# ox-vgg/wise

Measured on AMD Instinct MI355X. Metric: frames/sec embedded (ViT-B/32 bs=256) + queries/sec over 10M×512 index, 1/2/4/8 MI355X, higher is better.
Workload: dtype bf16; 1 GPU; OpenCLIP ViT-B/32 image tower (encode_image + L2 normalise), bs=256 frames per GPU, fp32 normalised frames resident in HBM -> [256,512] fp32 unit vectors; seeded random weights (no checkpoints offline); batches_in_flight=2, distinct_input_batches=4, layernorm_fold=True, global_batch=256, frames_per_gpu=256, parallelism=dp1, device=AMD Radeon Graphics

## Files before the change

### wise_amd/csrc/vit.hip

```cpp
#include "transformer.h"
#include "gemm_w4.h"

namespace wise {
#ifdef WISE_DEBUG_KNOBS
static int g_ablate = 0;
#else
constexpr int g_ablate = 0;
#endif

template <int NV>
__global__ __launch_bounds__(256) void layernorm_kernel(const float* x , const float* __restrict__ w,
                                                        const float* __restrict__ b, int rows, int W, float eps,
                                                        bf16_t* __restrict__ y, float* xo = nullptr) {
    const int lane = threadIdx.x & 63;
    const int row = blockIdx.x * 4 + (threadIdx.x >> 6);
    if (row >= rows) return;
    const int w4 = W >> 2;
    const float4* xr = reinterpret_cast<const float4*>(x + (size_t)row * W);
    float4 v[NV];
    float s = 0.f;
#pragma unroll
    for (int i = 0; i < NV; ++i) {
        const int c = i * 64 + lane;
        v[i] = (c < w4) ? xr[c] : make_float4(0.f, 0.f, 0.f, 0.f);
// ... 161 lines not shown
}

int layernorm_f32_dual(const float* x, const float* w, const float* b, int rows, int W, float eps, float* xo, bf16_t* y,
                       hipStream_t st) {
    WISE_CHECK_ARG(x && w && b && y && xo, "layernorm_dual: null pointer");
    WISE_CHECK_ARG(rows >= 0 && W > 128 && W % 4 == 0 && W <= 4096, "layernorm_dual: W=%d must be a multiple of 4 in (128, 4096]", W);
    if (rows == 0) return WISE_OK;
    const int nv = (W / 4 + 63) / 64;
    const dim3 grid((rows + 3) / 4), block(256);
#define LN_CASE(n) \
    case n: hipLaunchKernelGGL(layernorm_kernel<n>, grid, block, 0, st, x, w, b, rows, W, eps, y, xo); break;
    switch (nv) {
        LN_CASE(1) LN_CASE(2) LN_CASE(3) LN_CASE(4) LN_CASE(5) LN_CASE(6) LN_CASE(7) LN_CASE(8)
        LN_CASE(9) LN_CASE(10) LN_CASE(11) LN_CASE(12) LN_CASE(13) LN_CASE(14) LN_CASE(15) LN_CASE(16)
    }
#undef LN_CASE
    WISE_LAUNCH_CHECK("layernorm_kernel (dual)");
    return WISE_OK;
}

constexpr int V_RS = 144;
using short4v = __attribute__((ext_vector_type(4))) short;

template <int QT, bool MASK, int ND = 4>
__device__ __forceinline__ void softmax_block(f32x4 (&sacc)[4][QT], bf16x8 (&pf)[2][QT], f32x4 (&oacc)[ND][QT],
                                              float (&mrun)[QT], float (&lrun)[QT], int kbase, const int (&klim)[QT]) {
    const float sc = (ND == 4 ? 0.125f : 0.11180339887498948f) * 1.4426950408889634f;
#pragma unroll
    for (int qt = 0; qt < QT; ++qt) {
        float mx = -INFINITY;
#pragma unroll
        for (int kt = 0; kt < 4; ++kt)
#pragma unroll
            for (int r = 0; r < 4; ++r) {
                if (MASK && kbase + kt * 16 + r >= klim[qt]) sacc[kt][qt][r] = -INFINITY;
                mx = fmaxf(mx, sacc[kt][qt][r]);
            }
        mx = fmaxf(mx, __shfl_xor(mx, 16, 64));
        mx = fmaxf(mx, __shfl_xor(mx, 32, 64));
        const float mnew = fmaxf(mrun[qt], mx * sc);
        const float alpha = __builtin_amdgcn_exp2f(mrun[qt] - mnew);
        mrun[qt] = mnew;
        float ps = 0.f;
        float p[4][4];
#pragma unroll
        for (int kt = 0; kt < 4; ++kt)
#pragma unroll
            for (int r = 0; r < 4; ++r) {
                p[kt][r] = __builtin_amdgcn_exp2f(fmaf(sacc[kt][qt][r], sc, -mnew));
                ps += p[kt][r];
            }
        lrun[qt] = lrun[qt] * alpha + ps;
#pragma unroll
        for (int dt = 0; dt < ND; ++dt) {
            oacc[dt][qt][0] *= alpha; oacc[dt][qt][1] *= alpha;
            oacc[dt][qt][2] *= alpha; oacc[dt][qt][3] *= alpha;
        }
#pragma unroll
        for (int ks = 0; ks < 2; ++ks) {
            bf16x8 f;
#pragma unroll
            for (int r = 0; r < 4; ++r) {
                f[r] = (__bf16)p[2 * ks][r];
                f[4 + r] = (__bf16)p[2 * ks + 1][r];
            }
            pf[ks][qt] = f;
        }
    }
}

struct ClsRows {
    const bf16_t* hi = nullptr;
    long long lo_off = 0;
    bf16_t* hc = nullptr;
    long long lc_off = 0;
    const float* rs = nullptr;
    float* rs_c = nullptr;
    int* cnt = nullptr;
    int ncnt = 0;
};
__device__ __forceinline__ void cls_row_copy(const ClsRows& cr, int b, int T, int W, int lane) {
    const uint2* src = reinterpret_cast<const uint2*>(cr.hi + (size_t)b * T * W);
    uint2* dst = reinterpret_cast<uint2*>(cr.hc + (size_t)b * W);
    const long long so = cr.lo_off >> 2, dof = cr.lc_off >> 2;
    for (int c = lane; c < (W >> 2); c += 64) {
        dst[c] = src[c];
        dst[c + dof] = src[c + so];
    }
    if (cr.rs && lane == 0) cr.rs_c[b] = cr.rs[(size_t)b * T];
    if (b == 0)
        for (int c = lane; c < cr.ncnt; c += 64) cr.cnt[c] = 0;
}

template <int QT, bool CAUSAL, int DH = 64, bool PF = false, bool CLS = false>
__global__ __launch_bounds__(256, (QT == 2 && DH == 64 && !PF) ? 4 : 2) void attention_kernel(const bf16_t* __restrict__ qkv, int B, int T, int H,
                                                        bf16_t* __restrict__ o, const int* __restrict__ lens = nullptr,
                                                        const ClsRows cr = ClsRows()) {
    static_assert(!CLS || (QT == 1 && DH == 64 && !CAUSAL && !PF), "attention_kernel: the class-query form is QT = 1, DH = 64, no mask");
    constexpr int NS = (DH + 31) / 32, ND = DH / 16, VRS = DH * 2 + 16;
    __shared__ __attribute__((aligned(16))) unsigned char v_all[4][64 * VRS];
    const int lane = threadIdx.x & 63;
    const int wave = threadIdx.x >> 6;
    const int nqc = CLS ? 1 : (T + 16 * QT - 1) / (16 * QT);
    const long long item = (long long)blockIdx.x * 4 + wave;
    if (item >= (long long)B * H * nqc) return;
    const int qc = (int)(item % nqc);
    const int h = (int)((item / nqc) % H);
    const int b = (int)(item / ((long long)nqc * H));
    const int W = H * DH, W3 = 3 * W;
    const bf16_t* base = qkv + (size_t)b * T * W3;
    unsigned char* vimg = v_all[wave];
    const int l15 = lane & 15, g = lane >> 4;
    const int Tk = lens ? max(1, min(T, lens[b])) : T;

    const bf16x8 zero8 = {0, 0, 0, 0, 0, 0, 0, 0};
    bf16x8 qf[QT][NS];
#pragma unroll
    for (int qt = 0; qt < QT; ++qt) {
        int t = CLS ? 0 : qc * (16 * QT) + qt * 16 + l15;
        if (t >= T) t = T - 1;
#pragma unroll
        for (int s = 0; s < NS; ++s)
            qf[qt][s] = (s * 32 + g * 8 < DH) ? *reinterpret_cast<const bf16x8*>(base + (size_t)t * W3 + h * DH + s * 32 + g * 8)
                                              : zero8;
    }

    f32x4 oacc[ND][QT];
#pragma unroll
    for (int i = 0; i < ND; ++i)
#pragma unroll
        for (int j = 0; j < QT; ++j) oacc[i][j] = f32x4{0.f, 0.f, 0.f, 0.f};
    float mrun[QT], lrun[QT];
#pragma unroll
    for (int qt = 0; qt < QT; ++qt) { mrun[qt] = -INFINITY; lrun[qt] = 0.f; }

    const int q_last = min(T, (qc + 1) * (16 * QT)) - 1;
    const int nkb = CAUSAL ? (q_last >> 6) + 1 : (Tk + 63) >> 6;
    constexpr int CPR = DH / 8;
    auto load_k = [&](int kb, bf16x8 (&kf)[4][NS]) {
#pragma unroll
        for (int kt = 0; kt < 4; ++kt) {
            int t = kb * 64 + kt * 16 + l15;
            if (t >= Tk) t = Tk - 1;
#pragma unroll
            for (int s2 = 0; s2 < NS; ++s2)
                kf[kt][s2] = (s2 * 32 + g * 8 < DH) ? *reinterpret_cast<const bf16x8*>(base + (size_t)t * W3 + W + h * DH + s2 * 32 + g * 8)
                                                    : zero8;
        }
    };
    auto load_v = [&](int kb, uint4 (&vr)[CPR]) {
#pragma unroll
        for (int p = 0; p < CPR; ++p) {
            const int c = p * 64 + lane, key = c / CPR, part = c - key * CPR;
            int t = kb * 64 + key;
            const bool valid = t < Tk;
            if (!valid) t = Tk - 1;
            uint4 v = *reinterpret_cast<const uint4*>(base + (size_t)t * W3 + 2 * W + h * DH + part * 8);
            if (!valid) v = make_uint4(0u, 0u, 0u, 0u);
            vr[p] = v;
        }
// ... 57 lines not shown
            }
#pragma unroll
            for (int qt = 0; qt < QT; ++qt) {
                f32x4 c = f32x4{0.f, 0.f, 0.f, 0.f};
#pragma unroll
                for (int s2 = 0; s2 < NS; ++s2) c = __builtin_amdgcn_mfma_f32_16x16x32_bf16(kf[kt * KI][s2], qf[qt][s2], c, 0, 0, 0);
                sacc[kt][qt] = c;
            }
        }
        bf16x8 pf[2][QT];
        {
            int klim[QT];
#pragma unroll
            for (int qt = 0; qt < QT; ++qt) klim[qt] = CAUSAL ? min(T, qc * (16 * QT) + qt * 16 + l15 + 1) : Tk;
            if (CAUSAL || kb * 64 + 64 > Tk) {
#pragma unroll
                for (int qt = 0; qt < QT; ++qt)
#pragma unroll
                    for (int kt = 0; kt < 4; ++kt)
#pragma unroll
                        for (int r = 0; r < 4; ++r)
                            if (kb * 64 + kt * 16 + g * 4 + r >= klim[qt]) sacc[kt][qt][r] = -INFINITY;
            }
            softmax_block<QT, false, ND>(sacc, pf, oacc, mrun, lrun, kb * 64 + g * 4, klim);
        }
#pragma unroll
        for (int ks = 0; ks < 2; ++ks) {
#pragma unroll
            for (int dt = 0; dt < ND; ++dt) {
                const unsigned char* blk = vimg + (ks * 32 + g * 4 + (l15 >> 2)) * VRS + (dt * 16 + (l15 & 3) * 4) * 2;
                const short4v lo = __builtin_amdgcn_ds_read_tr16_b64_v4i16(
                    (__attribute__((address_space(3))) short4v*)(blk));
                const short4v hi = __builtin_amdgcn_ds_read_tr16_b64_v4i16(
                    (__attribute__((address_space(3))) short4v*)(blk + 16 * VRS));
                union { short8 s; bf16x8 f; } cv;
                cv.s = short8{lo[0], lo[1], lo[2], lo[3], hi[0], hi[1], hi[2], hi[3]};
#pragma unroll
                for (int qt = 0; qt < QT; ++qt)
                    oacc[dt][qt] = __builtin_amdgcn_mfma_f32_16x16x32_bf16(cv.f, pf[ks][qt], oacc[dt][qt], 0, 0, 0);
            }
        }
    }
#pragma unroll
    for (int qt = 0; qt < QT; ++qt) {
        float l = lrun[qt];
        l += __shfl_xor(l, 16, 64);
        l += __shfl_xor(l, 32, 64);
        const float inv = 1.f / l;
// ... 44 lines not shown
int attention_bf16(const bf16_t* qkv, int B, int T, int H, bf16_t* o, hipStream_t st, bool causal, int dh, const int* lens) {
    WISE_CHECK_ARG(qkv && o && B > 0 && T > 0 && H > 0, "attention: bad argument");
    WISE_CHECK_ARG(dh == 64 || (dh == 80 && !causal), "attention: head dim %d (64, or 80 without a mask)", dh);
    WISE_CHECK_ARG(!lens || (dh == 64 && !causal), "attention: per-sequence key counts go with head dim 64 and no causal mask");
    if (g_ablate & 4) return WISE_OK;
    if (dh == 80) {
        const long long items = (long long)B * H * ((T + 31) / 32);
        hipLaunchKernelGGL((attention_kernel<2, false, 80>), dim3((unsigned)((items + 3) / 4)), dim3(256), 0, st, qkv, B, T, H, o, (const int*)nullptr);
        WISE_LAUNCH_CHECK("attention_kernel");
        return WISE_OK;
    }
    if (!causal && g_attn_qt == 3) {
        const long long it3 = (long long)B * H * ((T + 47) / 48);
        hipLaunchKernelGGL((attention_kernel<3, false, 64, true>), dim3((unsigned)((it3 + 3) / 4)), dim3(256), 0, st, qkv, B, T, H, o, lens);
        WISE_LAUNCH_CHECK("attention_kernel");
        return WISE_OK;
    }
    if (!causal && g_attn_qt == 5) {
        const long long it2 = (long long)B * H * ((T + 31) / 32);
        hipLaunchKernelGGL((attention_kernel<2, false, 64, true>), dim3((unsigned)((it2 + 3) / 4)), dim3(256), 0, st, qkv, B, T, H, o, lens);
        WISE_LAUNCH_CHECK("attention_kernel");
        return WISE_OK;
    }
    const int qt = g_attn_qt ? (g_attn_qt == 4 ? 4 : 2) : (T <= 32 ? 2 : 4);
    const int nqc = (T + 16 * qt - 1) / (16 * qt);
    const long long items = (long long)B * H * nqc;
    const dim3 grid((unsigned)((items + 3) / 4)), block(256);
    if (causal) {
        if (qt == 4)
            hipLaunchKernelGGL((attention_kernel<4, true>), grid, block, 0, st, qkv, B, T, H, o, (const int*)nullptr);
        else
            hipLaunchKernelGGL((attention_kernel<2, true>), grid, block, 0, st, qkv, B, T, H, o, (const int*)nullptr);
    } else if (qt == 4)
        hipLaunchKernelGGL((attention_kernel<4, false>), grid, block, 0, st, qkv, B, T, H, o, lens);
    else
        hipLaunchKernelGGL((attention_kernel<2, false>), grid, block, 0, st, qkv, B, T, H, o, lens);
    WISE_LAUNCH_CHECK("attention_kernel");
    return WISE_OK;
}

#ifdef WISE_DEBUG_KNOBS
__device__ unsigned long long g_ao_stamps[12][8];
static int g_ao_dbg = 0;
#define AO_STAMP(k) do { if ((dbg & 8) && blockIdx.x == 0 && lane == 0) g_ao_stamps[wave][k] = __builtin_amdgcn_s_memtime(); } while (0)
#define AO_DBG_PARAM , int dbg
#define AO_DBG_ARG , g_ao_dbg
#else
#define AO_STAMP(k) do {} while (0)
#define AO_DBG_PARAM
#define AO_DBG_ARG
constexpr int dbg = 0;
#endif
template <int H>
__global__ __launch_bounds__(64 * H, 1) void attn_oproj_fold_kernel(const bf16_t* __restrict__ qkv, int T,
                                                                    const bf16_t* __restrict__ Wt, const float* __restrict__ bias,
                                                                    bf16_t* __restrict__ hi, long long lo_off,
// ... 379 lines not shown
#pragma unroll
                for (int e = 0; e < 4; ++e) {
                    acc[c8 * 8 + 2 * e] = fmaf(sc[i], __uint_as_float(w4[e] << 16), acc[c8 * 8 + 2 * e]);
                    acc[c8 * 8 + 2 * e + 1] = fmaf(sc[i], __uint_as_float(w4[e] & 0xFFFF0000u), acc[c8 * 8 + 2 * e + 1]);
                }
            }
        }
    }
    const float inv = 1.f / ps;
    float mine = 0.f;
#pragma unroll
    for (int j = 0; j < 64; ++j) {
        const float tot = wave_sum(acc[j]);
        if (lane == j) mine = tot * inv;
    }
    o[(size_t)b * W + h * 64 + lane] = f32_to_bf16(mine);
}

template <int NV>
__global__ __launch_bounds__(256) void embed_lnpre_kernel(const float* __restrict__ patch_out,
                                                          const float* __restrict__ cls, const float* __restrict__ pos,
                                                          const float* __restrict__ w, const float* __restrict__ bb,
                                                          int rows, int T, int W, float eps, float* __restrict__ x,
                                                          bf16_t* __restrict__ hcopy, float* __restrict__ rstd_out, long long lo_off) {
    const int lane = threadIdx.x & 63;
    const int row = blockIdx.x * 4 + (threadIdx.x >> 6);
    if (row >= rows) return;
    const int b = row / T, t = row % T;
    const int w4 = W >> 2;
    const float4* src = (t == 0) ? reinterpret_cast<const float4*>(cls)
                                 : reinterpret_cast<const float4*>(patch_out + ((size_t)b * (T - 1) + (t - 1)) * W);
    const float4* pr = reinterpret_cast<const float4*>(pos + (size_t)t * W);
    float4 v[NV];
    float s = 0.f;
#pragma unroll
    for (int i = 0; i < NV; ++i) {
        const int c = i * 64 + lane;
        if (c < w4) {
            float4 a = src[c], p = pr[c];
            v[i] = make_float4(a.x + p.x, a.y + p.y, a.z + p.z, a.w + p.w);
        } else
            v[i] = make_float4(0.f, 0.f, 0.f, 0.f);
        s += (v[i].x + v[i].y) + (v[i].z + v[i].w);
    }
    const float mean = wave_sum(s) / (float)W;
    float q = 0.f;
#pragma unroll
// ... 19 lines not shown
    }
    if (hcopy) {
        float s2 = 0.f;
#pragma unroll
        for (int i = 0; i < NV; ++i)
            if (i * 64 + lane < w4) s2 += (v[i].x + v[i].y) + (v[i].z + v[i].w);
        const float mean2 = wave_sum(s2) / (float)W;
        float q2 = 0.f;
#pragma unroll
        for (int i = 0; i < NV; ++i) {
            const int c = i * 64 + lane;
            if (c < w4) {
                float a0 = v[i].x - mean2, a1 = v[i].y - mean2, a2 = v[i].z - mean2, a3 = v[i].w - mean2;
                q2 += (a0 * a0 + a1 * a1) + (a2 * a2 + a3 * a3);
                const unsigned h0 = pack_bf16x2(v[i].x, v[i].y), h1 = pack_bf16x2(v[i].z, v[i].w);
                reinterpret_cast<uint2*>(hcopy + (size_t)row * W)[c] = make_uint2(h0, h1);
                reinterpret_cast<uint2*>(hcopy + lo_off + (size_t)row * W)[c] =
                    make_uint2(pack_bf16x2(v[i].x - __uint_as_float(h0 << 16), v[i].y - __uint_as_float(h0 & 0xffff0000u)),
                               pack_bf16x2(v[i].z - __uint_as_float(h1 << 16), v[i].w - __uint_as_float(h1 & 0xffff0000u)));
            }
        }
        const float r2 = rsqrtf(wave_sum(q2) / (float)W + eps);
        if (lane == 0) rstd_out[row] = r2;
    }
}

template <int NV>
__global__ __launch_bounds__(256) void cls_ln_kernel(const float* __restrict__ x, const float* __restrict__ w,
                                                     const float* __restrict__ b, int B, int T, int W, float eps,
                                                     bf16_t* __restrict__ y, const int* __restrict__ pos) {
    const int lane = threadIdx.x & 63;
    const int img = blockIdx.x * 4 + (threadIdx.x >> 6);
    if (img >= B) return;
    const int w4 = W >> 2;
    const float4* xr = reinterpret_cast<const float4*>(x + ((size_t)img * T + (pos ? pos[img] : 0)) * W);
    float4 v[NV];
    float s = 0.f;
#pragma unroll
    for (int i = 0; i < NV; ++i) {
        const int c = i * 64 + lane;
        v[i] = (c < w4) ? xr[c] : make_float4(0.f, 0.f, 0.f, 0.f);
        s += (v[i].x + v[i].y) + (v[i].z + v[i].w);
    }
    const float mean = wave_sum(s) / (float)W;
    float q = 0.f;
#pragma unroll
    for (int i = 0; i < NV; ++i) {
        if (i * 64 + lane < w4) {
            float a0 = v[i].x - mean, a1 = v[i].y - mean, a2 = v[i].z - mean, a3 = v[i].w - mean;
            q += (a0 * a0 + a1 * a1) + (a2 * a2 + a3 * a3);
        }
    }
    const float rstd = rsqrtf(wave_sum(q) / (float)W + eps);
    uint2* yr = reinterpret_cast<uint2*>(y + (size_t)img * W);
#pragma unroll
    for (int i = 0; i < NV; ++i) {
        const int c = i * 64 + lane;
        if (c < w4) {
            const float4 ww = reinterpret_cast<const float4*>(w)[c];
            const float4 bb = reinterpret_cast<const float4*>(b)[c];
            uint2 pk;
            pk.x = pack_bf16x2((v[i].x - mean) * rstd * ww.x + bb.x, (v[i].y - mean) * rstd * ww.y + bb.y);
            pk.y = pack_bf16x2((v[i].z - mean) * rstd * ww.z + bb.z, (v[i].w - mean) * rstd * ww.w + bb.w);
            yr[c] = pk;
// ... 36 lines not shown
    int rc;
    if (L > 0 && (rc = layernorm_f32_bf16(x, bw.pf + bw.ln1_w, bw.pf + bw.ln1_b, M, W, eps, h, st))) return rc;
    for (int l = 0; l < L; ++l) {
        const bf16_t* lwb = bw.wb + bw.per_layer_b * l;
        const float* lpf = bw.pf + bw.per_layer_f * l;
        if ((rc = gemm_bf16_rows(h, lwb + bw.in_proj, lpf + bw.in_b, Mp, Mv, 3 * W, W, 0, qkv, st, sk, sk_bytes))) return rc;
        if ((rc = attention_bf16(qkv, batch, T, H, h, st, causal, W / H))) return rc;
        if ((rc = gemm_resid_ln_rows(h, lwb + bw.out_proj, lpf + bw.out_b, Mp, Mv, M, W, W, x, lpf + bw.ln2_w, lpf + bw.ln2_b, eps,
                                     false, h, st, sk, sk_bytes)))
            return rc;
        if ((rc = gemm_bf16_rows(h, lwb + bw.c_fc, lpf + bw.fc_b, Mp, Mv, F, W, act == 0 ? 1 : (act == 1 ? 2 : 5), a, st, sk, sk_bytes))) return rc;
        if (l + 1 < L) {
            const float* npf = bw.pf + bw.per_layer_f * (l + 1);
            if ((rc = gemm_resid_ln_rows(a, lwb + bw.c_proj, lpf + bw.proj_b, Mp, Mv, M, W, F, x, npf + bw.ln1_w, npf + bw.ln1_b, eps,
                                         false, h, st, sk, sk_bytes)))
                return rc;
        } else if ((rc = gemm_bf16_rows(a, lwb + bw.c_proj, lpf + bw.proj_b, Mp, Mv, W, F, 3, x, st, sk, sk_bytes))) {
            return rc;
        }
    }
    return WISE_OK;
}

struct ClsTail {
    bf16_t* hc;
    bf16_t* o;
    float* stats;
    bf16_t* hb;
    int Bp;
};
static int transformer_blocks_fold(const BlockWeights& bw, int L, int W, int H, int F, int act, int batch, int T, float* x,
                                   bf16_t* h, bf16_t* qkv, bf16_t* a, float* stats, hipStream_t st, float eps, bool fuse_attn,
                                   const ClsTail* tail) {
    const int M = batch * T, Mp = (M + 255) / 256 * 256;
    int rc;
    float* rstd = stats;
    if (hipMemsetAsync(stats + Mp, 0, gemm_fold_counters_bytes(Mp), st) != hipSuccess) {
        set_error("vit_forward: memset of the fold counters failed");
        return WISE_E_INVALID;
    }
    bf16_t* hi = reinterpret_cast<bf16_t*>(x);
    const long long lo_off = (long long)Mp * W;
    bf16_t* ao = h;
    for (int l = 0; l < L; ++l) {
        const bf16_t* lwb = bw.wb + bw.per_layer_b * l;
        const float* lpf = bw.pf + bw.per_layer_f * l;
        if ((rc = gemm_fold_bf16(hi, lwb + bw.in_proj, lpf + bw.in_b, rstd, Mp, 3 * W, W, 0, qkv, st))) return rc;
        if (tail && l == L - 1) {
            const int Bp = tail->Bp;
            const long long lc_off = (long long)Bp * W;
            ClsRows cr;
            cr.hi = hi; cr.lo_off = lo_off; cr.hc = tail->hc; cr.lc_off = lc_off;
            cr.cnt = reinterpret_cast<int*>(tail->stats + Bp); cr.ncnt = (int)(gemm_fold_counters_bytes(Bp) / 4);
            if (fuse_attn) {
                if ((rc = attention_oproj_fold(qkv, batch, T, H, lwb + bw.out_proj, lpf + bw.out_b, hi, lo_off, rstd, eps, st))) return rc;
                cr.rs = rstd; cr.rs_c = tail->stats;
                hipLaunchKernelGGL(cls_rows_kernel, dim3((unsigned)((batch + 3) / 4)), dim3(256), 0, st, batch, T, W, cr);
                WISE_LAUNCH_CHECK("cls_rows_kernel");
            } else {
                if ((rc = attention_cls(qkv, batch, T, H, W, tail->o, cr, st))) return rc;
                if ((rc = gemm_fold_resid(tail->o, lwb + bw.out_proj, lpf + bw.out_b, Bp, W, W, tail->hc, lc_off, tail->stats, eps, st))) return rc;
            }
            if ((rc = gemm_fold_bf16(tail->hc, lwb + bw.c_fc, lpf + bw.fc_b, tail->stats, Bp, F, W, act == 0 ? 1 : (act == 1 ? 2 : 5), tail->o, st)))
                return rc;
            if ((rc = gemm_fold_resid(tail->o, lwb + bw.c_proj, lpf + bw.proj_b, Bp, W, F, tail->hc, lc_off, tail->stats, eps, st))) return rc;
            break;
        }
        if (fuse_attn) {
            if ((rc = attention_oproj_fold(qkv, batch, T, H, lwb + bw.out_proj, lpf + bw.out_b, hi, lo_off, rstd, eps, st))) return rc;
        } else {
            if ((rc = attention_bf16(qkv, batch, T, H, ao, st, false, W / H))) return rc;
            if ((rc = gemm_fold_resid(ao, lwb + bw.out_proj, lpf + bw.out_b, Mp, W, W, hi, lo_off, stats, eps, st))) return rc;
        }
        if ((rc = gemm_fold_bf16(hi, lwb + bw.c_fc, lpf + bw.fc_b, rstd, Mp, F, W, act == 0 ? 1 : (act == 1 ? 2 : 5), a, st))) return rc;
        if ((rc = gemm_fold_resid(a, lwb + bw.c_proj, lpf + bw.proj_b, Mp, W, F, hi, lo_off, stats, eps, st))) return rc;
    }
    return WISE_OK;
}

int pooled_ln(const float* x, const float* ln_w, const float* ln_b, int batch, int T, int W, const int* pos,
              bf16_t* hb, hipStream_t st, float eps) {
    const int nv = (W / 4 + 63) / 64;
    const dim3 grid((batch + 3) / 4), block(256);
#define CLS_CASE(n) case n: hipLaunchKernelGGL(cls_ln_kernel<n>, grid, block, 0, st, x, ln_w, ln_b, batch, T, W, eps, \
                                               hb, pos); break;
    switch (nv) {
        CLS_CASE(1) CLS_CASE(2) CLS_CASE(3) CLS_CASE(4) CLS_CASE(5) CLS_CASE(6) CLS_CASE(7) CLS_CASE(8)
        default: set_error("pooled_ln: width %d too large", W); return WISE_E_UNSUPPORTED;
    }
#undef CLS_CASE
    WISE_LAUNCH_CHECK("cls_ln_kernel");
    return WISE_OK;
}

int pooled_head(const float* x, const float* ln_w, const float* ln_b, const bf16_t* projT, int batch, int T, int W,
                int D, const int* pos, bf16_t* hb, float* e, float* out, hipStream_t st, float eps, const float* proj_bias) {
    const int Bp = (batch + 255) / 256 * 256;
    int rc;
    if ((rc = pooled_ln(x, ln_w, ln_b, batch, T, W, pos, hb, st, eps))) return rc;
    if ((rc = gemm_bf16(hb, projT, proj_bias, Bp, D, W, 4, e, st))) return rc;
    hipLaunchKernelGGL(l2norm_rows_kernel, dim3((batch + 3) / 4), dim3(256), 0, st, e, batch, D, out);
    WISE_LAUNCH_CHECK("l2norm_rows_kernel");
    return WISE_OK;
}

struct VitDims {
    int S, P, W, L, H, F, D, g, T, K, Kp, arch, fold;
};
static int vit_dims(const wise_vit_config* c, VitDims* d) {
    WISE_CHECK_ARG(c, "vit: null config");
    d->S = c->image_size; d->P = c->patch; d->W = c->width; d->L = c->layers; d->H = c->heads;
    d->F = c->mlp; d->D = c->embed_dim;
    WISE_CHECK_ARG(d->P > 0 && d->S > 0 && d->S % d->P == 0, "vit: image_size %d not a multiple of patch %d", d->S, d->P);
    WISE_CHECK_ARG(d->W > 0 && d->W % 128 == 0 && (d->H * 64 == d->W || d->H * 80 == d->W),
                   "vit: width %d must be heads * 64 (or heads * 80: ViT-H/14) and a multiple of 128", d->W);
    WISE_CHECK_ARG(d->F > 0 && d->F % 128 == 0, "vit: mlp %d must be a multiple of 128", d->F);
    WISE_CHECK_ARG(d->D > 0 && d->L >= 0 && d->W <= 4096 && d->W % 8 == 0, "vit: bad dims");
    WISE_CHECK_ARG(c->act >= 0 && c->act <= 2, "vit: act must be 0 (quick_gelu), 1 (gelu) or 2 (gelu, tanh form)");
    WISE_CHECK_ARG(c->arch == 0 || c->arch == 1, "vit: arch must be 0 (CLIP) or 1 (timm SigLIP: no class token, attention-pool head)");
    d->arch = c->arch;
    WISE_CHECK_ARG(c->ln_fold == 0 || ((c->ln_fold == 1 || c->ln_fold == 2) && c->arch == 0 && c->layers >= 1 && d->W >= 256),
                   "vit: ln_fold is 0, 1 or 2, and not 0 only for arch 0 with at least one block and width >= 256");
    d->fold = c->ln_fold;
    WISE_CHECK_ARG(d->arch == 0 || (d->D == d->W && d->H * 64 == d->W), "vit: the attention-pool head has no projection (embed_dim == width) and head dim 64");
    d->g = d->S / d->P; d->T = d->g * d->g + (d->arch == 0 ? 1 : 0); d->K = 3 * d->P * d->P; d->Kp = (d->K + 63) / 64 * 64;
    WISE_CHECK_ARG(d->arch == 0 || d->T <= 1024, "vit: the attention-pool head serves up to 1024 tokens");
// ... 63 lines not shown
#ifdef WISE_DEBUG_KNOBS
static int g_cls_tail = 1;
#else
constexpr int g_cls_tail = 1;
#endif

static bool cls_tail_layout(const VitDims& d, const VitWs& ws, int batch, unsigned char* wsb, ClsTail* t) {
    if (!d.fold || d.arch != 0 || !g_cls_tail || d.W != d.H * 64) return false;
    const size_t W = d.W, F = d.F, Bp = (size_t)(batch + 127) / 128 * 128, Bh = (size_t)(batch + 255) / 256 * 256;
    const size_t oa = align_up(Bp * std::max(W, F) * 2, 256), e_b = align_up(Bh * d.D * 4, 256);
    if (2 * Bp * W * 2 > ws.qkv - ws.h || oa + gemm_fold_stats_bytes((int)Bp, d.W) > ws.rstd - ws.a || (size_t)batch * W * 4 > ws.rstd - ws.a ||
        e_b + Bh * W * 2 > ws.a - ws.qkv)
        return false;
    t->hc = reinterpret_cast<bf16_t*>(wsb + ws.h);
    t->o = reinterpret_cast<bf16_t*>(wsb + ws.a);
    t->stats = reinterpret_cast<float*>(wsb + ws.a + oa);
    t->hb = reinterpret_cast<bf16_t*>(wsb + ws.qkv + e_b);
    t->Bp = (int)Bp;
    return true;
}

template <int NV>
static void launch_embed(const float* po, const float* cls, const float* pos, const float* w, const float* b, int rows,
                         int T, int W, float* x, hipStream_t st, bf16_t* hcopy, float* rstd_out, long long lo_off) {
    hipLaunchKernelGGL(embed_lnpre_kernel<NV>, dim3((rows + 3) / 4), dim3(256), 0, st, po, cls, pos, w, b, rows, T, W,
                       1e-5f, x, hcopy, rstd_out, lo_off);
}

__global__ __launch_bounds__(256) void hilo_rows_kernel(const bf16_t* __restrict__ hi, long long lo_off, int n, int stride, int W,
                                                        float* __restrict__ out, int ostride) {
    const long long i = (long long)blockIdx.x * 256 + threadIdx.x;
    if (i >= (long long)n * W) return;
    const int r = (int)(i / W), c = (int)(i % W);
    const size_t src = (size_t)r * stride * W + c;
    out[(size_t)r * ostride * W + c] = bf16_to_f32(hi[src]) + bf16_to_f32(hi[src + lo_off]);
}

static int vit_forward_part(const wise_vit_config* cfg, const VitDims& d, const VitOffsets& o, const bf16_t* wb,
                            const float* pf, const void* images, int in_kind, int batch, float* out,
                            unsigned char* wsb, hipStream_t st) {
    const VitWs ws = vit_ws(d, batch);
    float* x = reinterpret_cast<float*>(wsb + ws.x);
    bf16_t* h = reinterpret_cast<bf16_t*>(wsb + ws.h);
    bf16_t* qkv = reinterpret_cast<bf16_t*>(wsb + ws.qkv);
    bf16_t* a = reinterpret_cast<bf16_t*>(wsb + ws.a);
    float* patch_out = reinterpret_cast<float*>(wsb + ws.qkv);
    bf16_t* patches = a;
    const int W = d.W;
    int rc;
// ... 9 lines not shown
        else
            hipLaunchKernelGGL(patchify8_kernel<float>, dim3(blocks), dim3(256), 0, st,
                               reinterpret_cast<const float*>(images), total8, d.S, d.P, d.g, patches, nc);
    } else if (in_kind == WISE_VIT_IN_U8)
        hipLaunchKernelGGL(patchify_kernel<unsigned char>, dim3(ws.Mpatch), dim3(256), 0, st,
                           reinterpret_cast<const unsigned char*>(images), batch, d.S, d.P, d.g, d.Kp, patches, nc);
    else
        hipLaunchKernelGGL(patchify_kernel<float>, dim3(ws.Mpatch), dim3(256), 0, st,
                           reinterpret_cast<const float*>(images), batch, d.S, d.P, d.g, d.Kp, patches, nc);
    WISE_LAUNCH_CHECK("patchify_kernel");
    rc = gemm_bf16(patches, wb + o.conv1, nullptr, ws.Mpp, W, d.Kp, 4, patch_out, st);
    if (rc) return rc;
    if (d.arch == 1) {
        const long long total4 = (long long)ws.M * (W >> 2);
        hipLaunchKernelGGL(embed_pos_kernel, dim3((unsigned)((total4 + 255) / 256)), dim3(256), 0, st, patch_out, pf + o.pos,
                           total4, d.T, W, x);
        WISE_LAUNCH_CHECK("embed_pos_kernel");
    } else {

        const int nv = (W / 4 + 63) / 64;
        bf16_t* fh = d.fold ? reinterpret_cast<bf16_t*>(x) : nullptr;
        float* frs = d.fold ? reinterpret_cast<float*>(wsb + ws.rstd) : nullptr;
        const long long flo = (long long)ws.Mp * W;
        const float* cls = pf + o.cls; const float* pos = pf + o.pos;
        const float* lw = pf + o.ln_pre_w; const float* lb = pf + o.ln_pre_b;
        switch (nv) {
            case 1: launch_embed<1>(patch_out, cls, pos, lw, lb, ws.M, d.T, W, x, st, fh, frs, flo); break;
            case 2: launch_embed<2>(patch_out, cls, pos, lw, lb, ws.M, d.T, W, x, st, fh, frs, flo); break;
            case 3: launch_embed<3>(patch_out, cls, pos, lw, lb, ws.M, d.T, W, x, st, fh, frs, flo); break;
            case 4: launch_embed<4>(patch_out, cls, pos, lw, lb, ws.M, d.T, W, x, st, fh, frs, flo); break;
            case 5: launch_embed<5>(patch_out, cls, pos, lw, lb, ws.M, d.T, W, x, st, fh, frs, flo); break;
            case 6: launch_embed<6>(patch_out, cls, pos, lw, lb, ws.M, d.T, W, x, st, fh, frs, flo); break;
            case 7: launch_embed<7>(patch_out, cls, pos, lw, lb, ws.M, d.T, W, x, st, fh, frs, flo); break;
            case 8: launch_embed<8>(patch_out, cls, pos, lw, lb, ws.M, d.T, W, x, st, fh, frs, flo); break;
            default: set_error("vit_forward: width %d too large", W); return WISE_E_UNSUPPORTED;
        }
        WISE_LAUNCH_CHECK("embed_lnpre_kernel");
    }
    const BlockWeights bw = {wb + o.layer0_b, o.per_layer_b, o.in_proj, o.out_proj, o.c_fc, o.c_proj,
                             pf + o.layer0_f, o.per_layer_f, o.ln1_w, o.ln1_b, o.in_b, o.out_b, o.ln2_w, o.ln2_b,
                             o.fc_b, o.proj_b};
    ClsTail tail;
    const bool cls_tail = cls_tail_layout(d, ws, batch, wsb, &tail);
    if (d.fold) {
        if ((rc = transformer_blocks_fold(bw, d.L, W, d.H, d.F, cfg->act, batch, d.T, x, h, qkv, a,
                                          reinterpret_cast<float*>(wsb + ws.rstd), st, 1e-5f, d.fold == 2, cls_tail ? &tail : nullptr)))
            return rc;
    } else if ((rc = transformer_blocks(bw, d.L, W, d.H, d.F, cfg->act, batch, d.T, false, x, h, qkv, a, st,
                                        d.arch == 1 ? 1e-6f : 1e-5f)))
        return rc;
    if (d.arch == 1) {
        const int Bp = (batch + 255) / 256 * 256;
        if ((rc = layernorm_f32_bf16(x, pf + o.ln_post_w, pf + o.ln_post_b, ws.M, W, 1e-6f, h, st))) return rc;
        if ((rc = gemm_bf16(h, wb + o.h_kv, pf + o.h_kvb, ws.Mp, 2 * W, W, 0, qkv, st))) return rc;
        bf16_t* pooled = h;
        hipLaunchKernelGGL(map_pool_kernel, dim3(batch, d.H), dim3(64), 0, st, qkv, pf + o.hq, d.T, W, pooled);
        WISE_LAUNCH_CHECK("map_pool_kernel");
        float* y = reinterpret_cast<float*>(qkv);
        bf16_t* yn = a;
        bf16_t* hid = a + (size_t)Bp * W;
        if ((rc = gemm_bf16(pooled, wb + o.h_proj, pf + o.h_projb, Bp, W, W, 4, y, st))) return rc;
        if ((rc = layernorm_f32_bf16(y, pf + o.hn_w, pf + o.hn_b, batch, W, 1e-6f, yn, st))) return rc;
        if ((rc = gemm_bf16(yn, wb + o.h_fc1, pf + o.h_fc1b, Bp, d.F, W, 2, hid, st))) return rc;
        if ((rc = gemm_bf16(hid, wb + o.h_fc2, pf + o.h_fc2b, Bp, W, d.F, 3, y, st))) return rc;
        return l2norm_rows(y, batch, W, out, st);
    }
    if (d.fold) {
        float* xc = reinterpret_cast<float*>(a);
        const long long n = (long long)batch * W;
        if (cls_tail)
            hipLaunchKernelGGL(hilo_rows_kernel, dim3((unsigned)((n + 255) / 256)), dim3(256), 0, st, tail.hc, (long long)tail.Bp * W,
                               batch, 1, W, xc, 1);
        else
            hipLaunchKernelGGL(hilo_rows_kernel, dim3((unsigned)((n + 255) / 256)), dim3(256), 0, st, reinterpret_cast<const bf16_t*>(x),
                               (long long)ws.Mp * W, batch, d.T, W, xc, 1);
        WISE_LAUNCH_CHECK("hilo_rows_kernel");
        return pooled_head(xc, pf + o.ln_post_w, pf + o.ln_post_b, wb + o.projT, batch, 1, W, d.D, nullptr, cls_tail ? tail.hb : h,
                           reinterpret_cast<float*>(qkv), out, st);
    }
    if ((rc = pooled_head(x, pf + o.ln_post_w, pf + o.ln_post_b, wb + o.projT, batch, d.T, W, d.D, nullptr, h,
                          reinterpret_cast<float*>(qkv), out, st)))
        return rc;
    return WISE_OK;
}

constexpr int MAX_PARTS = 4;
static hipStream_t g_side[MAX_PARTS] = {nullptr, nullptr, nullptr, nullptr};
static hipEvent_t g_ev_fork = nullptr, g_ev_join[MAX_PARTS] = {nullptr, nullptr, nullptr, nullptr};
static int g_vit_streams = 2;
// ... 168 lines not shown
        } else {
            hipError_t e = hipMemcpyAsync(dp, wsb + base + ws.x, (size_t)ws.M * d.W * 4, hipMemcpyDeviceToDevice,
                                          (hipStream_t)stream);
            if (e != hipSuccess) { set_error("vit_tap_residual: %s", hipGetErrorString(e)); return (int)e; }
        }
        dp += (size_t)ws.M * d.W;
        base += ws.total;
    }
    return WISE_OK;
}

extern "C" int wise_layernorm_f32_bf16(const float* x, const float* w, const float* b, int rows, int W, float eps,
                                       uint16_t* y, void* stream) {
    return layernorm_f32_bf16(x, w, b, rows, W, eps, y, (hipStream_t)stream);
}

extern "C" int wise_attention_bf16(const uint16_t* qkv, int B, int T, int H, uint16_t* o, void* stream) {
    return attention_bf16(qkv, B, T, H, o, (hipStream_t)stream, false, 64);
}

#ifdef WISE_DEBUG_KNOBS
extern "C" int wise_debug_set_gemm_flags(int flags) { wise::g_ablate = flags & 6; return 0; }
extern "C" int wise_debug_set_vit_cls_tail(int on) { wise::g_cls_tail = on ? 1 : 0; return 0; }
extern "C" int wise_debug_attention_cls_bf16(const uint16_t* qkv, int B, int T, int H, uint16_t* o, void* stream) {
    return wise::attention_cls(qkv, B, T, H, H * 64, o, wise::ClsRows(), (hipStream_t)stream);
}
extern "C" int wise_debug_ao_set(int flags) { wise::g_ao_dbg = flags & 15; return 0; }
extern "C" int wise_debug_ao_stamps(unsigned long long* out) {
    return hipMemcpyFromSymbol(out, HIP_SYMBOL(wise::g_ao_stamps), sizeof(unsigned long long) * 96) == hipSuccess ? 0 : -1;
}
#endif
extern "C" int wise_attention_oproj_fold(const uint16_t* qkv, int B, int T, int H, const uint16_t* Wt, const float* bias,
                                         uint16_t* hi, int64_t lo_off, float* rstd, float eps, void* stream) {
    WISE_CHECK_ARG(lo_off >= (int64_t)B * T * H * 64, "attention_oproj_fold: lo_off %lld overlaps the hi rows", (long long)lo_off);
    return attention_oproj_fold(qkv, B, T, H, Wt, bias, hi, (long long)lo_off, rstd, eps, (hipStream_t)stream);
}

extern "C" int wise_attention_dh_bf16(const uint16_t* qkv, int B, int T, int H, int dh, uint16_t* o, void* stream) {
    return attention_bf16(qkv, B, T, H, o, (hipStream_t)stream, false, dh);
}
extern "C" int wise_attention_lens_bf16(const uint16_t* qkv, int B, int T, int H, const int32_t* lens, uint16_t* o, void* stream) {
    WISE_CHECK_ARG(lens, "attention_lens: null pointer");
    return attention_bf16(qkv, B, T, H, o, (hipStream_t)stream, false, 64, lens);
}
extern "C" int wise_attention_causal_bf16(const uint16_t* qkv, int B, int T, int H, uint16_t* o, void* stream) {
    return attention_bf16(qkv, B, T, H, o, (hipStream_t)stream, true, 64);
// ... 2 lines not shown
```

Measured before the change: 105,500 frames/s.

## Add single-key-block attention path and fold edge work into embed/pooled LN kernels

Adds an attention variant for non-causal T in (32,64] (ViT-B/32 has T=50) that skips online-softmax rescaling and accumulator init since only one key block exists, with a lower occupancy bound. Also zeroes the fold counters inside the embed/ln_pre kernel instead of a separate memset, and makes the pooled layernorm read hi/lo bf16 rows directly, removing the hilo_rows conversion kernel. These cut small kernel launches and per-block arithmetic, at the cost of more template variants and register pressure changes.

Result: no change. 106,300 frames/s, median of 6 (+0.8%).

```diff
diff --git a/wise_amd/csrc/vit.hip b/wise_amd/csrc/vit.hip
--- a/wise_amd/csrc/vit.hip
+++ b/wise_amd/csrc/vit.hip
@@ -207,7 +207,7 @@
 constexpr int V_RS = 144;
 using short4v = __attribute__((ext_vector_type(4))) short;
 
-template <int QT, bool MASK, int ND = 4>
+template <int QT, bool MASK, int ND = 4, bool ONE = false>
 __device__ __forceinline__ void softmax_block(f32x4 (&sacc)[4][QT], bf16x8 (&pf)[2][QT], f32x4 (&oacc)[ND][QT],
                                               float (&mrun)[QT], float (&lrun)[QT], int kbase, const int (&klim)[QT]) {
     const float sc = (ND == 4 ? 0.125f : 0.11180339887498948f) * 1.4426950408889634f;
@@ -223,9 +223,12 @@
             }
         mx = fmaxf(mx, __shfl_xor(mx, 16, 64));
         mx = fmaxf(mx, __shfl_xor(mx, 32, 64));
-        const float mnew = fmaxf(mrun[qt], mx * sc);
-        const float alpha = __builtin_amdgcn_exp2f(mrun[qt] - mnew);
-        mrun[qt] = mnew;
+        const float mnew = fmaxf(ONE ? -INFINITY : mrun[qt], mx * sc);
+        [[maybe_unused]] float alpha = 0.f;
+        if constexpr (!ONE) {
+            alpha = __builtin_amdgcn_exp2f(mrun[qt] - mnew);
+            mrun[qt] = mnew;
+        }
         float ps = 0.f;
         float p[4][4];
 #pragma unroll
@@ -235,11 +238,15 @@
                 p[kt][r] = __builtin_amdgcn_exp2f(fmaf(sacc[kt][qt][r], sc, -mnew));
                 ps += p[kt][r];
             }
-        lrun[qt] = lrun[qt] * alpha + ps;
-#pragma unroll
-        for (int dt = 0; dt < ND; ++dt) {
-            oacc[dt][qt][0] *= alpha; oacc[dt][qt][1] *= alpha;
-            oacc[dt][qt][2] *= alpha; oacc[dt][qt][3] *= alpha;
+        if constexpr (ONE) {
+            lrun[qt] = ps;
+        } else {
+            lrun[qt] = lrun[qt] * alpha + ps;
+#pragma unroll
+            for (int dt = 0; dt < ND; ++dt) {
+                oacc[dt][qt][0] *= alpha; oacc[dt][qt][1] *= alpha;
+                oacc[dt][qt][2] *= alpha; oacc[dt][qt][3] *= alpha;
+            }
         }
 #pragma unroll
         for (int ks = 0; ks < 2; ++ks) {
@@ -277,11 +284,12 @@
         for (int c = lane; c < cr.ncnt; c += 64) cr.cnt[c] = 0;
 }
 
-template <int QT, bool CAUSAL, int DH = 64, bool PF = false, bool CLS = false>
-__global__ __launch_bounds__(256, (QT == 2 && DH == 64 && !PF) ? 4 : 2) void attention_kernel(const bf16_t* __restrict__ qkv, int B, int T, int H,
+template <int QT, bool CAUSAL, int DH = 64, bool PF = false, bool CLS = false, bool ONE = false>
+__global__ __launch_bounds__(256, ONE ? 3 : (QT == 2 && DH == 64 && !PF) ? 4 : 2) void attention_kernel(const bf16_t* __restrict__ qkv, int B, int T, int H,
                                                         bf16_t* __restrict__ o, const int* __restrict__ lens = nullptr,
                                                         const ClsRows cr = ClsRows()) {
     static_assert(!CLS || (QT == 1 && DH == 64 && !CAUSAL && !PF), "attention_kernel: the class-query form is QT = 1, DH = 64, no mask");
+    static_assert(!ONE || (QT == 4 && DH == 64 && !CAUSAL && !PF && !CLS), "attention_kernel: the single-key-block form is QT = 4, DH = 64, no mask");
     constexpr int NS = (DH + 31) / 32, ND = DH / 16, VRS = DH * 2 + 16;
     __shared__ __attribute__((aligned(16))) unsigned char v_all[4][64 * VRS];
     const int lane = threadIdx.x & 63;
@@ -311,16 +319,19 @@
     }
 
     f32x4 oacc[ND][QT];
-#pragma unroll
-    for (int i = 0; i < ND; ++i)
-#pragma unroll
-        for (int j = 0; j < QT; ++j) oacc[i][j] = f32x4{0.f, 0.f, 0.f, 0.f};
+    auto zero_oacc = [&]() {
+#pragma unroll
+        for (int i = 0; i < ND; ++i)
+#pragma unroll
+            for (int j = 0; j < QT; ++j) oacc[i][j] = f32x4{0.f, 0.f, 0.f, 0.f};
+    };
+    if constexpr (!ONE) zero_oacc();
     float mrun[QT], lrun[QT];
 #pragma unroll
     for (int qt = 0; qt < QT; ++qt) { mrun[qt] = -INFINITY; lrun[qt] = 0.f; }
 
     const int q_last = min(T, (qc + 1) * (16 * QT)) - 1;
-    const int nkb = CAUSAL ? (q_last >> 6) + 1 : (Tk + 63) >> 6;
+    const int nkb = ONE ? 1 : CAUSAL ? (q_last >> 6) + 1 : (Tk + 63) >> 6;
     constexpr int CPR = DH / 8;
     auto load_k = [&](int kb, bf16x8 (&kf)[4][NS]) {
 #pragma unroll
@@ -424,8 +435,9 @@
                         for (int r = 0; r < 4; ++r)
                             if (kb * 64 + kt * 16 + g * 4 + r >= klim[qt]) sacc[kt][qt][r] = -INFINITY;
             }
-            softmax_block<QT, false, ND>(sacc, pf, oacc, mrun, lrun, kb * 64 + g * 4, klim);
-        }
+            softmax_block<QT, false, ND, ONE>(sacc, pf, oacc, mrun, lrun, kb * 64 + g * 4, klim);
+        }
+        if constexpr (ONE) zero_oacc();
 #pragma unroll
         for (int ks = 0; ks < 2; ++ks) {
 #pragma unroll
@@ -516,7 +528,8 @@
         WISE_LAUNCH_CHECK("attention_kernel");
         return WISE_OK;
     }
-    const int qt = g_attn_qt ? (g_attn_qt == 4 ? 4 : 2) : (T <= 32 ? 2 : 4);
+    const int qt = g_attn_qt ? (g_attn_qt == 4 || g_attn_qt == 6 ? 4 : 2) : (T <= 32 ? 2 : 4);
+    const bool one = !causal && qt == 4 && T > 32 && T <= 64 && g_attn_qt != 6;
     const int nqc = (T + 16 * qt - 1) / (16 * qt);
     const long long items = (long long)B * H * nqc;
     const dim3 grid((unsigned)((items + 3) / 4)), block(256);
@@ -525,7 +538,9 @@
             hipLaunchKernelGGL((attention_kernel<4, true>), grid, block, 0, st, qkv, B, T, H, o, (const int*)nullptr);
         else
             hipLaunchKernelGGL((attention_kernel<2, true>), grid, block, 0, st, qkv, B, T, H, o, (const int*)nullptr);
-    } else if (qt == 4)
+    } else if (one)
+        hipLaunchKernelGGL((attention_kernel<4, false, 64, false, false, true>), grid, block, 0, st, qkv, B, T, H, o, lens);
+    else if (qt == 4)
         hipLaunchKernelGGL((attention_kernel<4, false>), grid, block, 0, st, qkv, B, T, H, o, lens);
     else
         hipLaunchKernelGGL((attention_kernel<2, false>), grid, block, 0, st, qkv, B, T, H, o, lens);
@@ -951,7 +966,8 @@
                                                           const float* __restrict__ cls, const float* __restrict__ pos,
                                                           const float* __restrict__ w, const float* __restrict__ bb,
                                                           int rows, int T, int W, float eps, float* __restrict__ x,
-                                                          bf16_t* __restrict__ hcopy, float* __restrict__ rstd_out, long long lo_off) {
+                                                          bf16_t* __restrict__ hcopy, float* __restrict__ rstd_out, long long lo_off,
+                                                          int* __restrict__ cnt, int ncnt) {
     const int lane = threadIdx.x & 63;
     const int row = blockIdx.x * 4 + (threadIdx.x >> 6);
     if (row >= rows) return;
@@ -1017,24 +1033,36 @@
         }
         const float r2 = rsqrtf(wave_sum(q2) / (float)W + eps);
         if (lane == 0) rstd_out[row] = r2;
-    }
-}
-
-template <int NV>
-__global__ __launch_bounds__(256) void cls_ln_kernel(const float* __restrict__ x, const float* __restrict__ w,
+        if (cnt && row == 0)
+            for (int c = lane; c < ncnt; c += 64) cnt[c] = 0;
+    }
+}
+
+template <int NV, bool HILO = false>
+__global__ __launch_bounds__(256) void cls_ln_kernel(const void* __restrict__ xv, long long lo_off, const float* __restrict__ w,
                                                      const float* __restrict__ b, int B, int T, int W, float eps,
                                                      bf16_t* __restrict__ y, const int* __restrict__ pos) {
     const int lane = threadIdx.x & 63;
     const int img = blockIdx.x * 4 + (threadIdx.x >> 6);
     if (img >= B) return;
     const int w4 = W >> 2;
-    const float4* xr = reinterpret_cast<const float4*>(x + ((size_t)img * T + (pos ? pos[img] : 0)) * W);
+    const size_t roff = ((size_t)img * T + (pos ? pos[img] : 0)) * W;
     float4 v[NV];
     float s = 0.f;
 #pragma unroll
     for (int i = 0; i < NV; ++i) {
         const int c = i * 64 + lane;
-        v[i] = (c < w4) ? xr[c] : make_float4(0.f, 0.f, 0.f, 0.f);
+        if (c >= w4)
+            v[i] = make_float4(0.f, 0.f, 0.f, 0.f);
+        else if constexpr (HILO) {
+            const bf16_t* hr = reinterpret_cast<const bf16_t*>(xv) + roff;
+            const uint2 h = reinterpret_cast<const uint2*>(hr)[c], l = reinterpret_cast<const uint2*>(hr + lo_off)[c];
+            v[i] = make_float4(__uint_as_float(h.x << 16) + __uint_as_float(l.x << 16),
+                               __uint_as_float(h.x & 0xffff0000u) + __uint_as_float(l.x & 0xffff0000u),
+                               __uint_as_float(h.y << 16) + __uint_as_float(l.y << 16),
+                               __uint_as_float(h.y & 0xffff0000u) + __uint_as_float(l.y & 0xffff0000u));
+        } else
+            v[i] = reinterpret_cast<const float4*>(reinterpret_cast<const float*>(xv) + roff)[c];
         s += (v[i].x + v[i].y) + (v[i].z + v[i].w);
     }
     const float mean = wave_sum(s) / (float)W;
@@ -1117,6 +1145,11 @@
     return WISE_OK;
 }
 
+#ifdef WISE_DEBUG_KNOBS
+static bool g_fold_edges = true;
+#else
+constexpr bool g_fold_edges = true;
+#endif
 struct ClsTail {
     bf16_t* hc;
     bf16_t* o;
@@ -1130,7 +1163,7 @@
     const int M = batch * T, Mp = (M + 255) / 256 * 256;
     int rc;
     float* rstd = stats;
-    if (hipMemsetAsync(stats + Mp, 0, gemm_fold_counters_bytes(Mp), st) != hipSuccess) {
+    if (!g_fold_edges && hipMemsetAsync(stats + Mp, 0, gemm_fold_counters_bytes(Mp), st) != hipSuccess) {
         set_error("vit_forward: memset of the fold counters failed");
         return WISE_E_INVALID;
     }
@@ -1173,11 +1206,12 @@
     return WISE_OK;
 }
 
-int pooled_ln(const float* x, const float* ln_w, const float* ln_b, int batch, int T, int W, const int* pos,
-              bf16_t* hb, hipStream_t st, float eps) {
+template <bool HILO>
+static int pooled_ln_launch(const void* x, long long lo_off, const float* ln_w, const float* ln_b, int batch, int T, int W,
+                            const int* pos, bf16_t* hb, hipStream_t st, float eps) {
     const int nv = (W / 4 + 63) / 64;
     const dim3 grid((batch + 3) / 4), block(256);
-#define CLS_CASE(n) case n: hipLaunchKernelGGL(cls_ln_kernel<n>, grid, block, 0, st, x, ln_w, ln_b, batch, T, W, eps, \
+#define CLS_CASE(n) case n: hipLaunchKernelGGL((cls_ln_kernel<n, HILO>), grid, block, 0, st, x, lo_off, ln_w, ln_b, batch, T, W, eps, \
                                                hb, pos); break;
     switch (nv) {
         CLS_CASE(1) CLS_CASE(2) CLS_CASE(3) CLS_CASE(4) CLS_CASE(5) CLS_CASE(6) CLS_CASE(7) CLS_CASE(8)
@@ -1187,16 +1221,31 @@
     WISE_LAUNCH_CHECK("cls_ln_kernel");
     return WISE_OK;
 }
-
-int pooled_head(const float* x, const float* ln_w, const float* ln_b, const bf16_t* projT, int batch, int T, int W,
-                int D, const int* pos, bf16_t* hb, float* e, float* out, hipStream_t st, float eps, const float* proj_bias) {
+int pooled_ln(const float* x, const float* ln_w, const float* ln_b, int batch, int T, int W, const int* pos,
+              bf16_t* hb, hipStream_t st, float eps) {
+    return pooled_ln_launch<false>(x, 0, ln_w, ln_b, batch, T, W, pos, hb, st, eps);
+}
+
+static int pooled_proj(const bf16_t* hb, const bf16_t* projT, int batch, int W, int D, float* e, float* out, hipStream_t st,
+                       const float* proj_bias) {
     const int Bp = (batch + 255) / 256 * 256;
     int rc;
-    if ((rc = pooled_ln(x, ln_w, ln_b, batch, T, W, pos, hb, st, eps))) return rc;
     if ((rc = gemm_bf16(hb, projT, proj_bias, Bp, D, W, 4, e, st))) return rc;
     hipLaunchKernelGGL(l2norm_rows_kernel, dim3((batch + 3) / 4), dim3(256), 0, st, e, batch, D, out);
     WISE_LAUNCH_CHECK("l2norm_rows_kernel");
     return WISE_OK;
+}
+int pooled_head(const float* x, const float* ln_w, const float* ln_b, const bf16_t* projT, int batch, int T, int W,
+                int D, const int* pos, bf16_t* hb, float* e, float* out, hipStream_t st, float eps, const float* proj_bias) {
+    int rc;
+    if ((rc = pooled_ln(x, ln_w, ln_b, batch, T, W, pos, hb, st, eps))) return rc;
+    return pooled_proj(hb, projT, batch, W, D, e, out, st, proj_bias);
+}
+static int pooled_head_hilo(const bf16_t* hi, long long lo_off, const float* ln_w, const float* ln_b, const bf16_t* projT, int batch,
+                            int T, int W, int D, bf16_t* hb, float* e, float* out, hipStream_t st, float eps = 1e-5f) {
+    int rc;
+    if ((rc = pooled_ln_launch<true>(hi, lo_off, ln_w, ln_b, batch, T, W, nullptr, hb, st, eps))) return rc;
+    return pooled_proj(hb, projT, batch, W, D, e, out, st, nullptr);
 }
 
 struct VitDims {
@@ -1306,9 +1355,9 @@
 
 template <int NV>
 static void launch_embed(const float* po, const float* cls, const float* pos, const float* w, const float* b, int rows,
-                         int T, int W, float* x, hipStream_t st, bf16_t* hcopy, float* rstd_out, long long lo_off) {
+                         int T, int W, float* x, hipStream_t st, bf16_t* hcopy, float* rstd_out, long long lo_off, int* cnt, int ncnt) {
     hipLaunchKernelGGL(embed_lnpre_kernel<NV>, dim3((rows + 3) / 4), dim3(256), 0, st, po, cls, pos, w, b, rows, T, W,
-                       1e-5f, x, hcopy, rstd_out, lo_off);
+                       1e-5f, x, hcopy, rstd_out, lo_off, cnt, ncnt);
 }
 
 __global__ __launch_bounds__(256) void hilo_rows_kernel(const bf16_t* __restrict__ hi, long long lo_off, int n, int stride, int W,
@@ -1364,17 +1413,19 @@
         bf16_t* fh = d.fold ? reinterpret_cast<bf16_t*>(x) : nullptr;
         float* frs = d.fold ? reinterpret_cast<float*>(wsb + ws.rstd) : nullptr;
         const long long flo = (long long)ws.Mp * W;
+        int* fcnt = d.fold && g_fold_edges ? reinterpret_cast<int*>(frs + ws.Mp) : nullptr;
+        const int fncnt = (int)(gemm_fold_counters_bytes(ws.Mp) / 4);
         const float* cls = pf + o.cls; const float* pos = pf + o.pos;
         const float* lw = pf + o.ln_pre_w; const float* lb = pf + o.ln_pre_b;
         switch (nv) {
-            case 1: launch_embed<1>(patch_out, cls, pos, lw, lb, ws.M, d.T, W, x, st, fh, frs, flo); break;
-            case 2: launch_embed<2>(patch_out, cls, pos, lw, lb, ws.M, d.T, W, x, st, fh, frs, flo); break;
-            case 3: launch_embed<3>(patch_out, cls, pos, lw, lb, ws.M, d.T, W, x, st, fh, frs, flo); break;
-            case 4: launch_embed<4>(patch_out, cls, pos, lw, lb, ws.M, d.T, W, x, st, fh, frs, flo); break;
-            case 5: launch_embed<5>(patch_out, cls, pos, lw, lb, ws.M, d.T, W, x, st, fh, frs, flo); break;
-            case 6: launch_embed<6>(patch_out, cls, pos, lw, lb, ws.M, d.T, W, x, st, fh, frs, flo); break;
-            case 7: launch_embed<7>(patch_out, cls, pos, lw, lb, ws.M, d.T, W, x, st, fh, frs, flo); break;
-            case 8: launch_embed<8>(patch_out, cls, pos, lw, lb, ws.M, d.T, W, x, st, fh, frs, flo); break;
+            case 1: launch_embed<1>(patch_out, cls, pos, lw, lb, ws.M, d.T, W, x, st, fh, frs, flo, fcnt, fncnt); break;
+            case 2: launch_embed<2>(patch_out, cls, pos, lw, lb, ws.M, d.T, W, x, st, fh, frs, flo, fcnt, fncnt); break;
+            case 3: launch_embed<3>(patch_out, cls, pos, lw, lb, ws.M, d.T, W, x, st, fh, frs, flo, fcnt, fncnt); break;
+            case 4: launch_embed<4>(patch_out, cls, pos, lw, lb, ws.M, d.T, W, x, st, fh, frs, flo, fcnt, fncnt); break;
+            case 5: launch_embed<5>(patch_out, cls, pos, lw, lb, ws.M, d.T, W, x, st, fh, frs, flo, fcnt, fncnt); break;
+            case 6: launch_embed<6>(patch_out, cls, pos, lw, lb, ws.M, d.T, W, x, st, fh, frs, flo, fcnt, fncnt); break;
+            case 7: launch_embed<7>(patch_out, cls, pos, lw, lb, ws.M, d.T, W, x, st, fh, frs, flo, fcnt, fncnt); break;
+            case 8: launch_embed<8>(patch_out, cls, pos, lw, lb, ws.M, d.T, W, x, st, fh, frs, flo, fcnt, fncnt); break;
             default: set_error("vit_forward: width %d too large", W); return WISE_E_UNSUPPORTED;
         }
         WISE_LAUNCH_CHECK("embed_lnpre_kernel");
@@ -1407,6 +1458,13 @@
         if ((rc = gemm_bf16(hid, wb + o.h_fc2, pf + o.h_fc2b, Bp, W, d.F, 3, y, st))) return rc;
         return l2norm_rows(y, batch, W, out, st);
     }
+    if (d.fold && g_fold_edges) {
+        if (cls_tail)
+            return pooled_head_hilo(tail.hc, (long long)tail.Bp * W, pf + o.ln_post_w, pf + o.ln_post_b, wb + o.projT, batch, 1, W,
+                                    d.D, tail.hb, reinterpret_cast<float*>(qkv), out, st);
+        return pooled_head_hilo(reinterpret_cast<const bf16_t*>(x), (long long)ws.Mp * W, pf + o.ln_post_w, pf + o.ln_post_b,
+                                wb + o.projT, batch, d.T, W, d.D, h, reinterpret_cast<float*>(qkv), out, st);
+    }
     if (d.fold) {
         float* xc = reinterpret_cast<float*>(a);
         const long long n = (long long)batch * W;
@@ -1621,6 +1679,7 @@
 #ifdef WISE_DEBUG_KNOBS
 extern "C" int wise_debug_set_gemm_flags(int flags) { wise::g_ablate = flags & 6; return 0; }
 extern "C" int wise_debug_set_vit_cls_tail(int on) { wise::g_cls_tail = on ? 1 : 0; return 0; }
+extern "C" int wise_debug_set_vit_fold_edges(int on) { wise::g_fold_edges = on != 0; return 0; }
 extern "C" int wise_debug_attention_cls_bf16(const uint16_t* qkv, int B, int T, int H, uint16_t* o, void* stream) {
     return wise::attention_cls(qkv, B, T, H, H * 64, o, wise::ClsRows(), (hipStream_t)stream);
 }
```
